# NazirNayal8/RbA

Hardware: AMD Instinct MI355X
Metric: images/sec @1024x2048 Swin-B-1dl (RbA inference hot path) (higher is better)
Workload: dtype f32 (f16x3 split-MFMA GEMMs, fp32 accumulate)

## Files before the change

include/rba_hip.h:

```cpp
#ifndef RBA_HIP_H
#define RBA_HIP_H

#include <stdint.h>

#ifdef __cplusplus
extern "C" {
#endif

int rba_hip_version(void);

int rba_set_concurrent_streams(int n);

int rba_reduce_f32(const float* mask, const float* cls_prob, float* rba, float* sem_seg, int32_t* argmax,
                   int Q, int K, int64_t HW, int score_mode, void* stream);

int rba_reduce_ws_f32(const float* mask, const float* cls_prob, float* rba, float* sem_seg, int32_t* argmax, int Q, int K,
                      int64_t HW, int score_mode, void* workspace, void* stream);

int rba_reduce_up4_f32(const float* mask_lowres, const float* cls_prob, float* rba, float* sem_seg,
                       int32_t* argmax, int Q, int K, int h, int w, int crop_h, int crop_w, int score_mode, void* stream);

int rba_reduce_bwd_workspace_f32(int Q, int K, int64_t HW, int64_t* bytes);
int rba_reduce_bwd_f32(const float* mask, const float* cls_prob, const float* grad_score,
                       float* grad_mask , float* grad_prob ,
// ... 183 lines not shown

int rba_split_linear_f16x3_gn_moments_f32(const float* x, const void* weight_packed, const float* bias, float* out, int64_t M, int N, int K,
                                          int rows_per_image, int G, float* moments, void* stream);
int rba_conv3x3_nhwc_f16x3_split_in_gn_moments_f32(const void* x_frag, const void* weight_packed, const float* bias, float* out, int B, int H,
                                                   int W, int C, int N, int G, float* moments, void* stream);
int rba_group_norm_nhwc_merge_f32(const float* moments, float* mr, int B, int G, int splits, float eps, void* stream);

int rba_patch_im2col_u8(const uint8_t* image, float* out, int h, int w, int Hp, int Wp, const float* mean, const float* std, void* stream);
int rba_patch_im2col_f32(const float* image, float* out, int h, int w, int Hp, int Wp, const float* mean, const float* std, void* stream);

int rba_gaussian_blur_f32(const float* in, float* out, int H, int W, int kernel_size, float sigma, void* stream);

int rba_quad_mean_f32(const float* v, float* out, int64_t rows, int S, void* stream);
int rba_softmax_drop_last_f32(const float* logits, float* prob, int64_t rows, int K1, void* stream);

int rba_threshold_u8(const float* score, uint8_t* out, int64_t n, float threshold, void* stream);
int rba_morph3x3_u8(const uint8_t* in, uint8_t* out, int H, int W, int dilate, void* stream);
int rba_ccl4_roots_i32(const uint8_t* mask, int32_t* roots, int H, int W, void* stream);

int rba_bn_relu_conv1x1_f32(const float* x, const float* scale, const float* shift, const float* weight, const float* bias, float* out,
                            int B, int C, int O, int64_t P, void* stream);
int rba_resample_bilinear_ac_f32(const float* x, float* out, int C, int h, int w, int H, int W, void* stream);

typedef struct {
  const float* x_add;
  const void* packed;
  const float* bias;
  float* out;
  int N;
  int ld_out;
  int act;
} rba_token_linear_problem;
int rba_token_linear_pack_f16x2(const float* weight, void* packed, int N, int K, void* stream);
int rba_token_linear_f32(const float* x, const float* x_add, const void* packed, const float* bias, const float* residual,
                         const float* ln_weight, const float* ln_bias, float ln_eps, float* out, int64_t M, int N, int K, int act,
                         void* stream);
int rba_token_linear_multi_f32(const float* x, const rba_token_linear_problem* problems, int n_problems, int64_t M, int K, void* stream);

#define RBA_TTA_MAX_VIEWS 16
typedef struct {
  const float* sem[RBA_TTA_MAX_VIEWS];
  int h[RBA_TTA_MAX_VIEWS];
  int w[RBA_TTA_MAX_VIEWS];
  int flip[RBA_TTA_MAX_VIEWS];
} rba_tta_views;
int rba_tta_merge_f32(const rba_tta_views* views , int A, int K, int H, int W, int score_mode, float* score, float* sem_seg ,
                      int32_t* argmax , void* stream);

int rba_resize_u8_pil_bilinear(const uint8_t* in , uint8_t* out , uint8_t* tmp , int C, int h, int w,
                               int H, int W, const int32_t* kx, const int32_t* bx, int ksize_x, const int32_t* ky, const int32_t* by, int ksize_y,
                               int flip, void* stream);

int rba_confusion_accum(const int32_t* pred, const void* gt, int gt_bytes , int64_t n_pixels, int K,
                        int ignore_label , const uint8_t* lut , int64_t* conf ,
                        int64_t* bad , void* stream);

typedef struct {
  int enabled;
  int brightness;
  float beta;
  int order;
  int contrast;
  float contrast_alpha;
  int saturation;
  float saturation_alpha;
  int hue;
  int hue_delta;
} rba_train_view_color;
typedef struct {
// ... 25 lines not shown
```

rba_amd/_lib.py:

```python
import ctypes
import os

_HERE = os.path.dirname(os.path.abspath(__file__))
LIB_PATH = os.environ.get("RBA_HIP_LIB") or os.path.join(_HERE, "csrc", "librba_hip.so")
KNOBS_LIB_PATH = os.path.join(_HERE, "csrc", "librba_hip_knobs.so")

_i = ctypes.c_int
_i64 = ctypes.c_int64
_vp = ctypes.c_void_p

SIGNATURES = {
    "rba_hip_version": [],
    "rba_set_concurrent_streams": [_i],
    "rba_reduce_f32": [_vp, _vp, _vp, _vp, _vp, _i, _i, _i64, _i, _vp],
    "rba_reduce_ws_f32": [_vp, _vp, _vp, _vp, _vp, _i, _i, _i64, _i, _vp, _vp],
    "rba_reduce_up4_f32": [_vp, _vp, _vp, _vp, _vp, _i, _i, _i, _i, _i, _i, _i, _vp],
    "rba_reduce_bwd_workspace_f32": [_i, _i, _i64, _vp],
    "rba_reduce_bwd_f32": [_vp, _vp, _vp, _vp, _vp, _i, _i, _i64, _i, _vp, _i64, _vp],
    "rba_sem_seg_bwd_f32": [_vp, _vp, _vp, _vp, _vp, _i, _i, _i64, _vp, _i64, _vp],
    "rba_resample_bilinear_f32": [_vp, _vp, _vp, _i, _i, _i, _i, _i, _vp],
    "rba_ms_deform_attn_fwd_f32": [_vp, _vp, _vp, _vp, _vp, _vp, _i, _i, _i, _i, _i, _i, _i, _vp],
    "rba_ms_deform_attn_fwd_f64": [_vp, _vp, _vp, _vp, _vp, _vp, _i, _i, _i, _i, _i, _i, _i, _vp],
    "rba_ms_deform_attn_bwd_f32": [_vp, _vp, _vp, _vp, _vp, _vp, _vp, _vp, _vp, _i, _i, _i, _i, _i, _i, _i, _vp],
    "rba_ms_deform_attn_bwd_f64": [_vp, _vp, _vp, _vp, _vp, _vp, _vp, _vp, _vp, _i, _i, _i, _i, _i, _i, _i, _vp],
# ... 52 lines not shown
    "rba_swin_mlp_fused_ln_f16x3_f32": [_vp, _vp, _vp, ctypes.c_float, _vp, _vp, _vp, _vp, _i64, _i, _i, _vp],
    "rba_split_linear_f16x3_gelu_split_out": [_vp, _i, _vp, _vp, _vp, _i64, _i, _i, _vp],
    "rba_split_linear_nchw_out_f32": [_vp, _vp, _vp, _vp, _i64, _i, _i, _i, _vp],
    "rba_split_linear_nchw_out_f16x3_f32": [_vp, _vp, _vp, _vp, _i64, _i, _i, _i, _vp],
    "rba_split_linear_f16x3_gn_moments_f32": [_vp, _vp, _vp, _vp, _i64, _i, _i, _i, _i, _vp, _vp],
    "rba_conv3x3_nhwc_f16x3_split_in_gn_moments_f32": [_vp, _vp, _vp, _vp, _i, _i, _i, _i, _i, _i, _vp, _vp],
    "rba_group_norm_nhwc_merge_f32": [_vp, _vp, _i, _i, _i, ctypes.c_float, _vp],
    "rba_split_linear_nchw_out_gn_f16x3_f32": [_vp, _vp, _vp, _vp, _i, _i, _vp, _vp, _vp, _i64, _i, _i, _i, _vp],
    "rba_split_linear_nchw_out_gn_rows_f16x3_f32": [_vp, _vp, _vp, _vp, _i, _i, _vp, _i64, _vp, _i, _vp, _vp, _i, _i, _i, _i, _i, _vp],
    "rba_compose_query_operand_f16x2": [_vp, _vp, _vp, _vp, _vp, _i, _i, _i, _i, _vp],
    "rba_conv3x3_nhwc_f32": [_vp, _vp, _vp, _vp, _i, _i, _i, _i, _i, _vp],
    "rba_conv3x3_nhwc_f16x3_f32": [_vp, _vp, _vp, _vp, _i, _i, _i, _i, _i, _vp],
    "rba_conv3x3_nhwc_f16x3_split_in_f32": [_vp, _vp, _vp, _vp, _i, _i, _i, _i, _i, _vp],
    "rba_resample_bilinear_nhwc_split_out_f32": [_vp, _vp, _vp, _i, _i, _i, _i, _i, _i64, _vp],
    "rba_patch_im2col_u8": [_vp, _vp, _i, _i, _i, _i, _vp, _vp, _vp],
    "rba_patch_im2col_f32": [_vp, _vp, _i, _i, _i, _i, _vp, _vp, _vp],
    "rba_group_norm_nhwc_workspace_bytes": [_i, _i, _i, _i],
    "rba_group_norm_nhwc_f32": [_vp, _vp, _vp, _vp, _vp, _i, _i, _i, _i, ctypes.c_float, _i, _vp],
    "rba_resample_bilinear_nhwc_f32": [_vp, _vp, _vp, _i, _i, _i, _i, _i, _vp],
    "rba_bn_relu_conv1x1_f32": [_vp, _vp, _vp, _vp, _vp, _vp, _i, _i, _i, _i64, _vp],
    "rba_resample_bilinear_ac_f32": [_vp, _vp, _i, _i, _i, _i, _i, _vp],
    "rba_gaussian_blur_f32": [_vp, _vp, _i, _i, _i, ctypes.c_float, _vp],
    "rba_quad_mean_f32": [_vp, _vp, _i64, _i, _vp],
    "rba_softmax_drop_last_f32": [_vp, _vp, _i64, _i, _vp],
    "rba_threshold_u8": [_vp, _vp, _i64, ctypes.c_float, _vp],
    "rba_morph3x3_u8": [_vp, _vp, _i, _i, _i, _vp],
    "rba_ccl4_roots_i32": [_vp, _vp, _i, _i, _vp],
    "rba_add_layer_norm_f32": [_vp, _vp, _vp, _vp, _vp, _vp, _vp, _i64, _i, ctypes.c_float, _vp],
    "rba_add_layer_norm_frag_f32": [_vp, _vp, _vp, _vp, _vp, _vp, _vp, _i64, _i, ctypes.c_float, _vp],
    "rba_merge_layer_norm_f32": [_vp, _vp, _vp, _vp, _i, _i, _i, _i, ctypes.c_float, _vp],
    "rba_group_norm_workspace_bytes": [_i, _i, _i, _i],
    "rba_group_norm_f32": [_vp, _vp, _vp, _vp, _vp, _i, _i, _i, _i, ctypes.c_float, _i, _vp],
    "rba_token_linear_pack_f16x2": [_vp, _vp, _i, _i, _vp],
    "rba_token_linear_f32": [_vp, _vp, _vp, _vp, _vp, _vp, _vp, ctypes.c_float, _vp, _i64, _i, _i, _i, _vp],
    "rba_token_linear_multi_f32": [_vp, _vp, _i, _i64, _i, _vp],
}

class TokenLinearProblem(ctypes.Structure):
    _fields_ = [("x_add", ctypes.c_void_p), ("packed", ctypes.c_void_p), ("bias", ctypes.c_void_p), ("out", ctypes.c_void_p),
                ("N", ctypes.c_int), ("ld_out", ctypes.c_int), ("act", ctypes.c_int)]


TTA_MAX_VIEWS = 16


class TtaViews(ctypes.Structure):
    _fields_ = [("sem", ctypes.c_void_p * TTA_MAX_VIEWS), ("h", ctypes.c_int * TTA_MAX_VIEWS), ("w", ctypes.c_int * TTA_MAX_VIEWS),
                ("flip", ctypes.c_int * TTA_MAX_VIEWS)]


class TrainViewColor(ctypes.Structure):
    _fields_ = [("enabled", ctypes.c_int), ("brightness", ctypes.c_int), ("beta", ctypes.c_float), ("order", ctypes.c_int),
                ("contrast", ctypes.c_int), ("contrast_alpha", ctypes.c_float), ("saturation", ctypes.c_int), ("saturation_alpha", ctypes.c_float),
                ("hue", ctypes.c_int), ("hue_delta", ctypes.c_int)]


TRAIN_VIEW_POINTERS = ("img", "lab", "lut", "obj", "objmask", "kx", "bx", "ky", "by", "ny", "nx", "image", "sem_seg", "outlier_mask", "hist")
TRAIN_VIEW_INTS = ("h", "w", "bh", "bw", "py", "px", "new_h", "new_w", "ksize_x", "ksize_y", "y0", "x0", "ch", "cw", "flip", "pad_h", "pad_w",
                   "ignore_label", "ood_label")


class TrainView(ctypes.Structure):
    _fields_ = ([(n, ctypes.c_void_p) for n in TRAIN_VIEW_POINTERS] + [(n, ctypes.c_int) for n in TRAIN_VIEW_INTS] + [("color", TrainViewColor)])


EXPECTED_ABI = 191

# ... 81 lines not shown
```

rba_amd/csrc/swin_window_attn.hip:

```cpp
#include <stdlib.h>
#include "common.h"
#include "../../include/rba_hip.h"

namespace {

constexpr int CH = 16;

template <int HD>
__global__ __launch_bounds__(256) void swin_window_attn_kernel(const float* __restrict__ qkv, const float* __restrict__ qkv_bias,
                                                               const float* __restrict__ bias, float* __restrict__ out,
                                                               int H, int W, int Hp, int Wp, int nH, int ws, int shift, float scale) {
  extern __shared__ __attribute__((aligned(16))) float lds[];
  const int N = ws * ws;
  float* Ks = lds;
  float* Vs = lds + N * HD;
  int* rid = reinterpret_cast<int*>(lds + 2 * N * HD);
  const int wx = blockIdx.x, wy = blockIdx.y;
  const int h = blockIdx.z % nH, b = blockIdx.z / nH;
  const int C = nH * HD;
  const int64_t tok_stride = 3 * (int64_t)C;
  const float* qkv_b = qkv + (int64_t)b * H * W * tok_stride;

  for (int i = threadIdx.x; i < N * (HD / 4); i += blockDim.x) {
    const int t = i / (HD / 4), d4 = i % (HD / 4);
// ... 258 lines not shown

template <int NT, int WAVES>
int launch_mfma(const float* qkv, const float* qkv_bias, const float* bias, const float* bias_frag, float* out, int B, int H,
                int W, int Hp, int Wp, int nH, int ws, int shift, float scale, hipStream_t st) {
  const size_t shm = (size_t)(2 * NT * 16 * 36) * sizeof(float) + (size_t)(2 * NT * 16) * sizeof(int);
  const dim3 grid(Wp / ws, Hp / ws, B * nH), block(64 * WAVES);
  if (bias_frag)
    hipLaunchKernelGGL((swin_window_attn_mfma_kernel<NT, WAVES, true>), grid, block, shm, st, qkv, qkv_bias, bias_frag, out,
                       H, W, Hp, Wp, nH, ws, shift, scale);
  else
    hipLaunchKernelGGL((swin_window_attn_mfma_kernel<NT, WAVES, false>), grid, block, shm, st, qkv, qkv_bias, bias, out,
                       H, W, Hp, Wp, nH, ws, shift, scale);
  return rba_launch_status();
}

__global__ void swin_bias_fragments_kernel(const float* __restrict__ bias, float* __restrict__ frag, int nH, int N, int NT) {
  const int64_t total = (int64_t)nH * NT * NT * 256;
  for (int64_t i = (int64_t)blockIdx.x * blockDim.x + threadIdx.x; i < total; i += (int64_t)gridDim.x * blockDim.x) {
    const int r = (int)(i & 3), lane = (int)((i >> 2) & 63);
    int64_t j = i >> 8;
    const int c = (int)(j % NT); j /= NT;
    const int strip = (int)(j % NT);
    const int h = (int)(j / NT);
    const int q = strip * 16 + (lane & 15), k = c * 16 + 4 * (lane >> 4) + r;
    frag[i] = (q < N && k < N) ? bias[((int64_t)h * N + q) * N + k] : 0.f;
  }
}

}

#include "swin_window_attn_h3.h"

RBA_KNOB(rba_k5_wpe, 6);

namespace {
template <int NT, int WAVES>
int launch_h3(const float* qkv, const float* qkv_bias, const float* bias, const float* bias_frag, float* out, int B, int H, int W,
              int Hp, int Wp, int nH, int ws, int shift, float scale, hipStream_t st, bool split_out = false) {
  const size_t shm = (size_t)(4 * NT * 16 * 64) + (size_t)(2 * NT * 16) * sizeof(int);
  const dim3 grid(Wp / ws, Hp / ws, B * nH), block(64 * WAVES);
#define K5H_LAUNCH(FRAG, SOUT, WPE, BIAS) hipLaunchKernelGGL((swin_window_attn_h3_kernel<NT, WAVES, FRAG, SOUT, WPE>), grid, block, shm, st, qkv, qkv_bias, BIAS, out, H, W, Hp, Wp, nH, ws, shift, scale)
  const int w = rba_k5_wpe;
  if (split_out && !bias_frag) return (int)hipErrorInvalidValue;
  if (split_out) {
    if (w == 5) K5H_LAUNCH(true, true, 5, bias_frag); else if (w == 7) K5H_LAUNCH(true, true, 7, bias_frag); else K5H_LAUNCH(true, true, 6, bias_frag);
  } else if (bias_frag) {
    if (w == 5) K5H_LAUNCH(true, false, 5, bias_frag); else if (w == 7) K5H_LAUNCH(true, false, 7, bias_frag); else K5H_LAUNCH(true, false, 6, bias_frag);
  } else {
    if (w == 5) K5H_LAUNCH(false, false, 5, bias); else if (w == 7) K5H_LAUNCH(false, false, 7, bias); else K5H_LAUNCH(false, false, 6, bias);
  }
#undef K5H_LAUNCH
  return rba_launch_status();
}

}

extern "C" int64_t rba_swin_bias_fragments_elems(int nH, int ws) {
  if (nH <= 0 || ws <= 0 || ws * ws > 256) return 0;
  const int64_t NT = (ws * ws + 15) / 16;
  return (int64_t)nH * NT * NT * 256;
}

extern "C" int rba_swin_bias_fragments_f32(const float* bias, float* frag, int nH, int ws, void* stream) {
  RBA_CHECK_ARG(bias && frag && nH >= 1 && ws >= 1 && ws * ws <= 256);
  rba_begin();
  const int N = ws * ws, NT = (N + 15) / 16;
  const int64_t total = (int64_t)nH * NT * NT * 256;
  hipLaunchKernelGGL(swin_bias_fragments_kernel, dim3((unsigned)((total + 255) / 256)), dim3(256), 0, (hipStream_t)stream, bias,
                     frag, nH, N, NT);
  return rba_launch_status();
}

extern "C" int rba_swin_window_attn_f32(const float* qkv, const float* qkv_bias, const float* bias, const float* bias_frag,
                                        float* out, int B, int H, int W, int nH, int hd, int ws, int shift, void* stream) {
// ... 42 lines not shown
```

rba_amd/csrc/swin_window_attn_h3.h:

```cpp
#pragma once

#ifdef K5H_TIMING
#define K5H_DBG_PARAM , unsigned long long* __restrict__ dbg
#define K5H_STAMP(i)                                                                                                              \
  do {                                                                                                                            \
    __builtin_amdgcn_sched_barrier(0);                                                                                            \
    if ((threadIdx.x & 63) == 0)                                                                                                  \
      dbg[((((int64_t)blockIdx.z * gridDim.y + blockIdx.y) * gridDim.x + blockIdx.x) * WAVES + (threadIdx.x >> 6)) * 12 + (i)] = wall_clock64(); \
    __builtin_amdgcn_sched_barrier(0);                                                                                            \
  } while (0)
#define K5H_WAIT_VM() __builtin_amdgcn_s_waitcnt(0x0070 | 0x0F00 | 0xC000 * 0)
#define K5H_SINK(x) asm volatile("" ::"s"(__builtin_amdgcn_readfirstlane(__builtin_bit_cast(int, (x)))))
#elif defined(K5H_ABLATE)
#define K5H_DBG_PARAM , int ablate
#define K5H_STAMP(i)
#define K5H_WAIT_VM()
#define K5H_SINK(x)
#else
#define K5H_DBG_PARAM
#define K5H_STAMP(i)
#define K5H_WAIT_VM()
#define K5H_SINK(x)
#endif

namespace {

typedef _Float16 k5h_f16x8 __attribute__((ext_vector_type(8)));
typedef _Float16 k5h_f16x2 __attribute__((ext_vector_type(2)));
typedef __fp16 k5h_h4 __attribute__((__vector_size__(4 * sizeof(__fp16))));
typedef uint32_t k5h_u32x4 __attribute__((ext_vector_type(4)));

template <bool SCALED>
__device__ __forceinline__ void k5h_split2(float a, float b, uint32_t& h, uint32_t& l) {
  const k5h_f16x2 hv = {(_Float16)a, (_Float16)b};
  h = __builtin_bit_cast(uint32_t, hv);
  const float m = SCALED ? -2048.0f : -1.0f;
  const float a2 = SCALED ? a * 2048.0f : a, b2 = SCALED ? b * 2048.0f : b;
  uint32_t r;
  asm("v_fma_mixlo_f16 %0, %1, %2, %3 op_sel_hi:[1,0,0]" : "=v"(r) : "v"(h), "v"(m), "v"(a2));
  asm("v_fma_mixhi_f16 %0, %1, %2, %3 op_sel:[1,0,0] op_sel_hi:[1,0,0]" : "+v"(r) : "v"(h), "v"(m), "v"(b2));
  l = r;
}

template <int NT, int WAVES, bool FRAG, bool SOUT = false, int WPE = 5>
__global__ __launch_bounds__(64 * WAVES) __attribute__((amdgpu_waves_per_eu(WPE, 8))) void swin_window_attn_h3_kernel(
    const float* __restrict__ qkv, const float* __restrict__ qkv_bias, const float* __restrict__ bias, float* __restrict__ out,
    int H, int W, int Hp, int Wp, int nH, int ws, int shift, float scale K5H_DBG_PARAM) {
  K5H_STAMP(0);
#ifdef K5H_ABLATE
  if (((ablate >> 3) & 0xff) && ((((blockIdx.z * gridDim.y + blockIdx.y) * gridDim.x + blockIdx.x) >> 8) & 1)) {
    const unsigned long long t0 = wall_clock64();
    while (wall_clock64() - t0 < (unsigned long long)(((ablate >> 3) & 0xff) * 50)) __builtin_amdgcn_s_sleep(4);
  }
#endif
  constexpr int HD = 32, NP = NT * 16, PL = NP * 64;
  if (NT == 9) ws = 12;
  extern __shared__ __attribute__((aligned(16))) unsigned char k5h_lds[];
  unsigned char* Kh = k5h_lds;
  int* tok = reinterpret_cast<int*>(k5h_lds + 4 * PL);
  int* rid = tok + NP;
  const int N = NT == 9 ? 144 : ws * ws;
  int wx = blockIdx.x, wy = blockIdx.y, hz = blockIdx.z;
#ifdef K5H_ABLATE
  if (ablate & 0x4000) {
    const int L = (blockIdx.z * gridDim.y + blockIdx.y) * gridDim.x + blockIdx.x;
    const int hh = L % nH, wl = L / nH;
    wx = wl % (int)gridDim.x;
    wy = (wl / (int)gridDim.x) % (int)gridDim.y;
    hz = (wl / (int)(gridDim.x * gridDim.y)) * nH + hh;
  }
#endif
  const bool need_mask = shift > 0 && (wy == (int)gridDim.y - 1 || wx == (int)gridDim.x - 1);
  const int h = hz % nH, b = hz / nH;
  const int C = nH * HD;
  const int64_t tok_stride = 3 * (int64_t)C;
  const float* qkv_b = qkv + (int64_t)b * H * W * tok_stride;
  const float* qb = qkv_bias + h * HD;

  constexpr int NIT = (NP * (HD / 4) + 64 * WAVES - 1) / (64 * WAVES);
  float4 kk4[NIT], vv4[NIT];
  int tkv[NIT], rgv[NIT];
#pragma unroll
  for (int it = 0; it < NIT; ++it) {
    const int i = threadIdx.x + it * 64 * WAVES;
    const int t = i >> 3, d4 = i & 7;
    kk4[it] = vv4[it] = make_float4(0.f, 0.f, 0.f, 0.f);
    tkv[it] = -2;
    rgv[it] = -1;
    if (i < NP * (HD / 4) && t < N) {
      const int r = wy * ws + t / ws, c = wx * ws + t % ws;
      int rr = r + shift, cc = c + shift;
      rr = rr >= Hp ? rr - Hp : rr;
      cc = cc >= Wp ? cc - Wp : cc;
#ifdef K5H_ABLATE
      if (ablate & 2) rr = H;
#endif
      if (rr < H && cc < W) {
        tkv[it] = rr * W + cc;
        const float* p = qkv_b + (int64_t)tkv[it] * tok_stride + h * HD + d4 * 4;
        kk4[it] = *reinterpret_cast<const float4*>(p + C);
        vv4[it] = *reinterpret_cast<const float4*>(p + 2 * C);
      } else {
        tkv[it] = -1;
        kk4[it] = *reinterpret_cast<const float4*>(qb + C + d4 * 4);
        vv4[it] = *reinterpret_cast<const float4*>(qb + 2 * C + d4 * 4);
      }
      const int hid = r < Hp - ws ? 0 : (r < Hp - shift ? 1 : 2);
      const int wid = c < Wp - ws ? 0 : (c < Wp - shift ? 1 : 2);
      rgv[it] = hid * 3 + wid;
    }
  }
  float4 q_a = make_float4(0.f, 0.f, 0.f, 0.f), q_b = q_a;
  {
    const int qt0 = (threadIdx.x >> 6) * 16 + (threadIdx.x & 15), kq = (threadIdx.x & 63) >> 4;
    if ((threadIdx.x >> 6) < NT && qt0 < N) {
      const int r = wy * ws + qt0 / ws, c = wx * ws + qt0 % ws;
      int rr = r + shift, cc = c + shift;
      rr = rr >= Hp ? rr - Hp : rr;
      cc = cc >= Wp ? cc - Wp : cc;
#ifdef K5H_ABLATE
      if (ablate & 2) rr = H;
#endif
      const float4* p = (rr < H && cc < W) ? reinterpret_cast<const float4*>(qkv_b + (int64_t)(rr * W + cc) * tok_stride + h * HD + kq * 8)
                                           : reinterpret_cast<const float4*>(qb + kq * 8);
      q_a = p[0];
      q_b = p[1];
    }
  }
  K5H_STAMP(1);
  K5H_WAIT_VM();
  K5H_STAMP(2);
#pragma unroll
  for (int it = 0; it < NIT; ++it) {
    const int i = threadIdx.x + it * 64 * WAVES;
    if (i >= NP * (HD / 4)) break;
    const int t = i >> 3, d4 = i & 7;
    uint32_t h0, l0, h1, l1;
    const int tq = (t >> 2) & 3;
    const int perm = (0x1320 >> (4 * tq)) & 3;
    k5h_split2<false>(kk4[it].x, kk4[it].y, h0, l0);
    k5h_split2<false>(kk4[it].z, kk4[it].w, h1, l1);
    const int ko = t * 64 + (((d4 >> 1) ^ perm) * 16) + (d4 & 1) * 8;
    *reinterpret_cast<uint2*>(Kh + ko) = make_uint2(h0, h1);
    *reinterpret_cast<uint2*>(Kh + PL + ko) = make_uint2(l0, l1);
    k5h_split2<true>(vv4[it].x, vv4[it].y, h0, l0);
    k5h_split2<true>(vv4[it].z, vv4[it].w, h1, l1);
    const int vo = t * 64 + (((d4 >> 2) ^ (tq & 1)) * 32) + (d4 & 3) * 8;
    *reinterpret_cast<uint2*>(Kh + 2 * PL + vo) = make_uint2(h0, h1);
    *reinterpret_cast<uint2*>(Kh + 3 * PL + vo) = make_uint2(l0, l1);
    if (d4 == 0) { tok[t] = tkv[it]; rid[t] = rgv[it]; }
  }
  K5H_STAMP(3);
  __syncthreads();
  K5H_STAMP(4);

  const int lane = threadIdx.x & 63, wave = threadIdx.x >> 6;
  const int l15 = lane & 15, kk = lane >> 4;
  const bool vec_bias = (N & 3) == 0;
  const int kfrag = l15 * 64 + ((kk ^ ((0x1320 >> (4 * ((l15 >> 2) & 3))) & 3)) * 16);
  const int vfrag = (4 * kk + (l15 >> 2)) * 64 + (l15 & 3) * 8;
// ... 196 lines not shown
```

rba_amd/csrc/token_linear.hip:

```cpp
#include "common.h"
#include "../../include/rba_hip.h"

namespace {

typedef _Float16 tl_f16x8 __attribute__((ext_vector_type(8)));
typedef float tl_f32x4 __attribute__((ext_vector_type(4)));

struct TlProblem {
  const float* x_add;
  const rba_u32x4* wp;
  const float* bias;
  float* out;
  int N;
  int ld;
  int act;
};
struct TlProblems {
  TlProblem p[3];
};

__global__ void token_linear_pack_kernel(const float* __restrict__ w, rba_u32x4* __restrict__ packed, int N, int K) {
  const int KB = K >> 5;
  const int64_t total = (int64_t)((N + 15) >> 4) * KB * 128;
  for (int64_t i = (int64_t)blockIdx.x * blockDim.x + threadIdx.x; i < total; i += (int64_t)gridDim.x * blockDim.x) {
// ... 205 lines not shown
        for (int r = 0; r < 4; ++r) y[r] = (val[rt][i][r] - mean[rt]) * rstd * g[r] + be[r];
        *reinterpret_cast<f32x4*>(p.out + (int64_t)row[rt] * p.N + n) = y;
      }
    }
  }
}

RBA_KNOB(rba_token_rt, 0);

template <bool LN>
int launch_token_linear(const float* x, const TlProblems& ps, int nprob, const float* residual, const float* ln_w, const float* ln_b, float eps,
                        int M, int K, hipStream_t st) {
  int nmax = 0;
  for (int i = 0; i < nprob; ++i) nmax = ps.p[i].N > nmax ? ps.p[i].N : nmax;
  const int ctw = (((nmax + 15) >> 4) + TLW - 1) / TLW;
  const bool two = rba_token_rt == 2 || (rba_token_rt == 0 && K >= 512 && M >= 4096);
  const dim3 grid((unsigned)((M + (two ? 31 : 15)) / (two ? 32 : 16)), (unsigned)nprob);
#define RBA_TL(C)                                                                                                                     \
  if (two) hipLaunchKernelGGL((token_linear_kernel<C, LN, 2>), grid, dim3(64 * TLW), 0, st, x, ps, residual, ln_w, ln_b, eps, M, K);   \
  else hipLaunchKernelGGL((token_linear_kernel<C, LN, 1>), grid, dim3(64 * TLW), 0, st, x, ps, residual, ln_w, ln_b, eps, M, K)
  switch (ctw) {
    case 1: RBA_TL(1); break;
    case 2: RBA_TL(2); break;
    case 3: RBA_TL(3); break;
    case 4: RBA_TL(4); break;
    default: return (int)hipErrorInvalidValue;
  }
#undef RBA_TL
  return rba_launch_status();
}

inline bool tl_aligned(const void* p) { return (reinterpret_cast<uintptr_t>(p) & 15) == 0; }

}

extern "C" {

int rba_token_linear_pack_f16x2(const float* weight, void* packed, int N, int K, void* stream) {
  RBA_CHECK_ARG(weight && packed && N >= 1 && K >= 32 && K % 32 == 0 && tl_aligned(packed));
  rba_begin();
  const int64_t total = (int64_t)((N + 15) >> 4) * (K >> 5) * 128;
  const int blocks = (int)((total + 255) / 256 < 4096 ? (total + 255) / 256 : 4096);
  hipLaunchKernelGGL(token_linear_pack_kernel, dim3(blocks), dim3(256), 0, (hipStream_t)stream, weight, reinterpret_cast<rba_u32x4*>(packed), N, K);
  return rba_launch_status();
}

int rba_token_linear_f32(const float* x, const float* x_add, const void* packed, const float* bias, const float* residual,
                         const float* ln_weight, const float* ln_bias, float ln_eps, float* out, int64_t M, int N, int K, int act,
                         void* stream) {
  RBA_CHECK_ARG(x && packed && out && M >= 0 && M < ((int64_t)1 << 31) - 16 && N >= 1 && N <= 256 && K >= 32 && K % 32 == 0);
  RBA_CHECK_ARG(act == 0 || act == 2);
  RBA_CHECK_ARG(tl_aligned(x) && tl_aligned(x_add) && tl_aligned(packed) && tl_aligned(out) && tl_aligned(bias) && N % 4 == 0);
  const bool ln = ln_weight != nullptr;
  RBA_CHECK_ARG(!ln || (residual && ln_bias && N % 16 == 0 && act == 0 && tl_aligned(residual) && tl_aligned(ln_weight) && tl_aligned(ln_bias)));
  RBA_CHECK_ARG(ln || !residual);
  if (M == 0) return 0;
  rba_begin();
  TlProblems ps{};
  ps.p[0] = TlProblem{x_add, reinterpret_cast<const rba_u32x4*>(packed), bias, out, N, N, act};
  if (ln) return launch_token_linear<true>(x, ps, 1, residual, ln_weight, ln_bias, ln_eps, (int)M, K, (hipStream_t)stream);
  return launch_token_linear<false>(x, ps, 1, nullptr, nullptr, nullptr, 0.f, (int)M, K, (hipStream_t)stream);
}

int rba_token_linear_multi_f32(const float* x, const rba_token_linear_problem* problems, int n_problems, int64_t M, int K, void* stream) {
  RBA_CHECK_ARG(x && problems && n_problems >= 1 && n_problems <= 3 && M >= 0 && M < ((int64_t)1 << 31) - 16 && K >= 32 && K % 32 == 0 && tl_aligned(x));
  TlProblems ps{};
  for (int i = 0; i < n_problems; ++i) {
    const rba_token_linear_problem& q = problems[i];
    RBA_CHECK_ARG(q.packed && q.out && q.N >= 1 && q.N <= 256 && q.N % 4 == 0 && q.ld_out >= q.N && q.ld_out % 4 == 0 && (q.act == 0 || q.act == 2));
    RBA_CHECK_ARG(tl_aligned(q.x_add) && tl_aligned(q.packed) && tl_aligned(q.bias) && tl_aligned(q.out));
    ps.p[i] = TlProblem{q.x_add, reinterpret_cast<const rba_u32x4*>(q.packed), q.bias, q.out, q.N, q.ld_out, q.act};
  }
  if (M == 0) return 0;
  rba_begin();
  return launch_token_linear<false>(x, ps, n_problems, nullptr, nullptr, nullptr, 0.f, (int)M, K, (hipStream_t)stream);
}

}
```

rba_amd/ops.py:

```python
import contextlib
import ctypes
import threading
import functools
import math
import os

import torch

from . import _lib
from ._lib import RbaHipError
from .lru import derived


def _stream():
    return torch.cuda.current_stream().cuda_stream


def _launch(name, *args, stream=None):
    code = getattr(_lib.load(), name)(*args, torch.cuda.current_stream().cuda_stream if stream is None else stream)
    if code:
        _lib.check(code, name)


def _query(name, *args):
# ... 1389 lines not shown
    _vec(bias, "bias", N, optional=True)
    splits = H * W // 128
    out = torch.empty((B, H, W, N), dtype=torch.float32, device=x.device)
    mom = torch.empty((B, num_groups, splits, 3), dtype=torch.float32, device=x.device)
    _launch("rba_conv3x3_nhwc_f16x3_split_in_gn_moments_f32", xp, _p(planes), _p(bias), _p(out), B, H, W, C, N, int(num_groups), _p(mom))
    return out, _merge_gn_moments(mom, B, int(num_groups), splits, eps)


def split_linear_nchw_out_takes_gn(planes, rows_per_image, K, num_groups):
    return planes.dtype == torch.float16 and rows_per_image % 128 == 0 and K % num_groups == 0 and (K // num_groups) % 4 == 0 and K % 32 == 0


@_hip_op
def split_linear_nchw_out_gn(x, mr, weight, bias_gn, num_groups, relu, planes, bias, rows_per_image, out_features=None):
    _chk(x, "x", dim=2)
    _chk(mr, "mr", dim=3)
    M, K = x.shape
    N, _ = _packed(planes, K, out_features, bf16x6=False)
    if rows_per_image < 1 or M % rows_per_image or not split_linear_nchw_out_takes_gn(planes, rows_per_image, K, num_groups):
        raise RbaHipError("split_linear_nchw_out_gn needs x [B*P, K], P % 128 == 0 and (K / G) % 4 == 0")
    B = M // rows_per_image
    if tuple(mr.shape) != (B, num_groups, 2):
        raise RbaHipError("mr must be [B, G, 2]")
    _vec(weight, "weight", K)
    _vec(bias_gn, "bias_gn", K)
    _vec(bias, "bias", N, optional=True)
    out = torch.empty((B, N, rows_per_image), dtype=torch.float32, device=x.device)
    _launch("rba_split_linear_nchw_out_gn_f16x3_f32", _p(x), _p(mr), _p(weight), _p(bias_gn), int(num_groups), int(bool(relu)), _p(planes), _p(bias), _p(out),
            M, N, K, rows_per_image)
    return out


COMPOSED_MASK_HEAD = os.environ.get("RBA_COMPOSED_MASK_HEAD", "1") != "0"


class RowIndex:
    __slots__ = ("data", "rows_per_image")

    def __init__(self, data, rows_per_image):
        self.data, self.rows_per_image = data, rows_per_image


def row_index(idx, rows_per_image):
    if not isinstance(idx, torch.Tensor) or not idx.is_cuda or idx.dtype not in (torch.int32, torch.int64) or idx.dim() != 2 or idx.numel() == 0:
        raise RbaHipError("row_index needs a HIP int32 / int64 tensor [B, R]")
    lo, hi = int(idx.min()), int(idx.max())
    if lo < 0 or hi >= rows_per_image:
        raise RbaHipError(f"row_index: values must lie in [0, {rows_per_image}), got [{lo}, {hi}]")
    return RowIndex(idx.to(torch.int32).contiguous(), int(rows_per_image))


def _image_planes(planes, K, out_features, B):
    if planes.dim() != 7:
        return _packed(planes, K, out_features, bf16x6=False)[0], 0
    _chk(planes, "planes", dtype=torch.float16, dim=7)
    if planes.shape[0] != B:
        raise RbaHipError(f"per-image planes must be [B = {B}, ...], got {tuple(planes.shape)}")
    return _packed(planes[0], K, out_features, bf16x6=False)[0], planes.stride(0) * 2


@_hip_op
def split_linear_nchw_out_gn_rows(x, mr, weight, bias_gn, num_groups, relu, planes, bias, rows_per_image, out_features=None, rows=None):
    _chk(x, "x", dim=2)
    _chk(mr, "mr", dim=3)
    M, K = x.shape
    P = int(rows_per_image)
# ... 100 lines not shown

def _token_planes(lin):
    w = lin.weight

    def build():
        w2 = w.detach().contiguous()
        _chk(w2, "weight", dim=2)
        N, K = w2.shape
        packed = torch.empty((((N + 15) // 16) * (K // 32) * 128, 4), dtype=torch.int32, device=w.device)
        _launch("rba_token_linear_pack_f16x2", _p(w2), _p(packed), N, K)
        return packed

    return derived(lin, "token_planes", (w,), build)


@_hip_op
def token_linear(x, lin, x_add=None, use_bias=True, relu=False, residual=None, norm=None):
    _chk(x, "x")
    N, K = lin.weight.shape
    if x.shape[-1] != K or not token_linear_ok(N, K):
        raise RbaHipError("token_linear: x [..., K] with K % 32 == 0, N <= 256 and the f16x3 mode (see token_linear_ok)")
    M = x.numel() // K
    _shaped(x_add, "x_add", x.shape, optional=True)
    bias = _vec(lin.bias if use_bias else None, "bias", N, optional=True)
    if (residual is None) != (norm is None):
        raise RbaHipError("token_linear: residual and norm come together")
    ln_w, ln_b, ln_eps, act = 0, 0, 0.0, 2 if relu else 0
    if norm is not None:
        _chk(residual, "residual")
        if tuple(residual.shape) != tuple(x.shape[:-1]) + (N,) or N % 16 or relu or norm.weight.numel() != N:
            raise RbaHipError("token_linear(norm=...): residual [..., N], N % 16 == 0, no activation")
        ln_w, ln_b, ln_eps = _p(norm.weight), _p(norm.bias), float(norm.eps)
    out = torch.empty(tuple(x.shape[:-1]) + (N,), dtype=torch.float32, device=x.device)
    _launch("rba_token_linear_f32", _p(x), _p(x_add), _p(_token_planes(lin)), _p(bias), _p(residual), ln_w, ln_b, ln_eps, _p(out), M, N, K, act)
    return out


@_hip_op
def token_linear_multi(x, specs):
    _chk(x, "x")
    K = x.shape[-1]
    M = x.numel() // K if K else 0
    lead = tuple(x.shape[:-1])
    if not 1 <= len(specs) <= 3:
        raise RbaHipError("token_linear_multi: one to three problems")
    arr = (_lib.TokenLinearProblem * len(specs))()
    outs, keep = [], []
    for i, (lin, x_add, out, col0, relu) in enumerate(specs):
        N, K_ = lin.weight.shape
        if K_ != K or not token_linear_ok(N, K) or N % 4:
            raise RbaHipError("token_linear_multi: weights [N <= 256, N % 4 == 0, K] with x's K % 32 == 0 (see token_linear_ok)")
        _shaped(x_add, "x_add", x.shape, optional=True)
        _vec(lin.bias, "bias", N, optional=True)
        if out is None:
            out, col0 = torch.empty(lead + (N,), dtype=torch.float32, device=x.device), 0
        else:
            _chk(out, "out")
            if tuple(out.shape[:-1]) != lead or col0 % 4 or col0 + N > out.shape[-1] or out.shape[-1] % 4:
                raise RbaHipError("token_linear_multi: out [..., ld] with ld % 4 == 0 and a column slice col0 % 4 == 0 inside it")
        planes = _token_planes(lin)
        keep.append(planes)
        arr[i] = _lib.TokenLinearProblem(_p(x_add) or None, _p(planes), _p(lin.bias) or None, out.data_ptr() + 4 * col0, N, out.shape[-1], 2 if relu else 0)
        outs.append(out)
    _launch("rba_token_linear_multi_f32", _p(x), ctypes.byref(arr), len(specs), M, K)
    return outs


# ... 177 lines not shown
```

Measured before the change: 151.6.

## Add split-K token linear path and 32-bit-offset gather in Swin window attention

Adds a split-K MFMA kernel plus a separate reduce+bias+residual+LayerNorm finish kernel for token_linear when M is small, N=256 and K>=1024, so the GEMM fills more of the GPU. Partial sums go to a workspace that the host sizes through a new query function. It also adds a GATHER32 variant of the Swin window-attention load that uses 32-bit byte offsets and a row-strided thread mapping for full 12x12 windows, and uses inline -1.0 constants in the unscaled fma_mix path. The costs are extra workspace traffic, one more launch, and a gather path that only covers specific shapes.

After: 152.2, median of 6. Within noise of the previous version (+0.4%).

```diff
diff --git a/include/rba_hip.h b/include/rba_hip.h
--- a/include/rba_hip.h
+++ b/include/rba_hip.h
@@ -239,9 +239,10 @@
   int act;
 } rba_token_linear_problem;
 int rba_token_linear_pack_f16x2(const float* weight, void* packed, int N, int K, void* stream);
+int64_t rba_token_linear_workspace_bytes(int64_t M, int N, int K, int has_ln, int has_x_add);
 int rba_token_linear_f32(const float* x, const float* x_add, const void* packed, const float* bias, const float* residual,
                          const float* ln_weight, const float* ln_bias, float ln_eps, float* out, int64_t M, int N, int K, int act,
-                         void* stream);
+                         void* workspace, int64_t workspace_bytes, void* stream);
 int rba_token_linear_multi_f32(const float* x, const rba_token_linear_problem* problems, int n_problems, int64_t M, int K, void* stream);
 
 #define RBA_TTA_MAX_VIEWS 16
diff --git a/rba_amd/_lib.py b/rba_amd/_lib.py
--- a/rba_amd/_lib.py
+++ b/rba_amd/_lib.py
@@ -108,7 +108,8 @@
     "rba_group_norm_workspace_bytes": [_i, _i, _i, _i],
     "rba_group_norm_f32": [_vp, _vp, _vp, _vp, _vp, _i, _i, _i, _i, ctypes.c_float, _i, _vp],
     "rba_token_linear_pack_f16x2": [_vp, _vp, _i, _i, _vp],
-    "rba_token_linear_f32": [_vp, _vp, _vp, _vp, _vp, _vp, _vp, ctypes.c_float, _vp, _i64, _i, _i, _i, _vp],
+    "rba_token_linear_workspace_bytes": [_i64, _i, _i, _i, _i],
+    "rba_token_linear_f32": [_vp, _vp, _vp, _vp, _vp, _vp, _vp, ctypes.c_float, _vp, _i64, _i, _i, _i, _vp, _i64, _vp],
     "rba_token_linear_multi_f32": [_vp, _vp, _i, _i64, _i, _vp],
 }
 
diff --git a/rba_amd/csrc/swin_window_attn.hip b/rba_amd/csrc/swin_window_attn.hip
--- a/rba_amd/csrc/swin_window_attn.hip
+++ b/rba_amd/csrc/swin_window_attn.hip
@@ -314,6 +314,7 @@
 #include "swin_window_attn_h3.h"
 
 RBA_KNOB(rba_k5_wpe, 6);
+RBA_KNOB(rba_k5_gather, 0);
 
 namespace {
 template <int NT, int WAVES>
@@ -321,7 +322,12 @@
               int Hp, int Wp, int nH, int ws, int shift, float scale, hipStream_t st, bool split_out = false) {
   const size_t shm = (size_t)(4 * NT * 16 * 64) + (size_t)(2 * NT * 16) * sizeof(int);
   const dim3 grid(Wp / ws, Hp / ws, B * nH), block(64 * WAVES);
-#define K5H_LAUNCH(FRAG, SOUT, WPE, BIAS) hipLaunchKernelGGL((swin_window_attn_h3_kernel<NT, WAVES, FRAG, SOUT, WPE>), grid, block, shm, st, qkv, qkv_bias, BIAS, out, H, W, Hp, Wp, nH, ws, shift, scale)
+  const bool g32 = rba_k5_gather == 0 && (int64_t)H * W * 3 * nH * 32 * (int64_t)sizeof(float) < ((int64_t)1 << 32);
+#define K5H_LAUNCH(FRAG, SOUT, WPE, BIAS)                                                                                                                        \
+  do {                                                                                                                                                           \
+    if (g32) hipLaunchKernelGGL((swin_window_attn_h3_kernel<NT, WAVES, FRAG, SOUT, WPE, true>), grid, block, shm, st, qkv, qkv_bias, BIAS, out, H, W, Hp, Wp, nH, ws, shift, scale); \
+    else hipLaunchKernelGGL((swin_window_attn_h3_kernel<NT, WAVES, FRAG, SOUT, WPE, false>), grid, block, shm, st, qkv, qkv_bias, BIAS, out, H, W, Hp, Wp, nH, ws, shift, scale);   \
+  } while (0)
   const int w = rba_k5_wpe;
   if (split_out && !bias_frag) return (int)hipErrorInvalidValue;
   if (split_out) {
diff --git a/rba_amd/csrc/swin_window_attn_h3.h b/rba_amd/csrc/swin_window_attn_h3.h
--- a/rba_amd/csrc/swin_window_attn_h3.h
+++ b/rba_amd/csrc/swin_window_attn_h3.h
@@ -37,12 +37,17 @@
   const float m = SCALED ? -2048.0f : -1.0f;
   const float a2 = SCALED ? a * 2048.0f : a, b2 = SCALED ? b * 2048.0f : b;
   uint32_t r;
-  asm("v_fma_mixlo_f16 %0, %1, %2, %3 op_sel_hi:[1,0,0]" : "=v"(r) : "v"(h), "v"(m), "v"(a2));
-  asm("v_fma_mixhi_f16 %0, %1, %2, %3 op_sel:[1,0,0] op_sel_hi:[1,0,0]" : "+v"(r) : "v"(h), "v"(m), "v"(b2));
+  if constexpr (SCALED) {
+    asm("v_fma_mixlo_f16 %0, %1, %2, %3 op_sel_hi:[1,0,0]" : "=v"(r) : "v"(h), "v"(m), "v"(a2));
+    asm("v_fma_mixhi_f16 %0, %1, %2, %3 op_sel:[1,0,0] op_sel_hi:[1,0,0]" : "+v"(r) : "v"(h), "v"(m), "v"(b2));
+  } else {
+    asm("v_fma_mixlo_f16 %0, %1, -1.0, %2 op_sel_hi:[1,0,0]" : "=v"(r) : "v"(h), "v"(a2));
+    asm("v_fma_mixhi_f16 %0, %1, -1.0, %2 op_sel:[1,0,0] op_sel_hi:[1,0,0]" : "+v"(r) : "v"(h), "v"(b2));
+  }
   l = r;
 }
 
-template <int NT, int WAVES, bool FRAG, bool SOUT = false, int WPE = 5>
+template <int NT, int WAVES, bool FRAG, bool SOUT = false, int WPE = 5, bool GATHER32 = false>
 __global__ __launch_bounds__(64 * WAVES) __attribute__((amdgpu_waves_per_eu(WPE, 8))) void swin_window_attn_h3_kernel(
     const float* __restrict__ qkv, const float* __restrict__ qkv_bias, const float* __restrict__ bias, float* __restrict__ out,
     int H, int W, int Hp, int Wp, int nH, int ws, int shift, float scale K5H_DBG_PARAM) {
@@ -80,6 +85,56 @@
   constexpr int NIT = (NP * (HD / 4) + 64 * WAVES - 1) / (64 * WAVES);
   float4 kk4[NIT], vv4[NIT];
   int tkv[NIT], rgv[NIT];
+  float4 q_a = make_float4(0.f, 0.f, 0.f, 0.f), q_b = q_a;
+  if constexpr (GATHER32) {
+    static_assert(NT == 9 && WAVES <= NT && (8 * WAVES) % 12 == 0 && (NP * (HD / 4)) % (64 * WAVES) == 0,
+                  "GATHER32: full 12 x 12 windows, a thread's pieces whole window rows apart");
+    constexpr int RSTEP = 8 * WAVES / 12;
+    const uint32_t tokb = 12u * (uint32_t)C;
+    const uint32_t rowb = tokb * (uint32_t)W;
+    const char* kbase = reinterpret_cast<const char*>(qkv_b + h * HD + C);
+    const char* vbase = reinterpret_cast<const char*>(qkv_b + h * HD + 2 * C);
+    const int t0 = threadIdx.x >> 3, d4 = threadIdx.x & 7;
+    const int r0 = wy * 12 + t0 / 12, c = wx * 12 + t0 % 12;
+    int cc = c + shift;
+    cc = cc >= Wp ? cc - Wp : cc;
+    const bool colok = cc < W;
+    const int wid = c < Wp - 12 ? 0 : (c < Wp - shift ? 1 : 2);
+    const uint32_t coff = (uint32_t)cc * tokb + (uint32_t)d4 * 16u;
+#pragma unroll
+    for (int it = 0; it < NIT; ++it) {
+      const int r = r0 + it * RSTEP;
+      int rr = r + shift;
+      rr = rr >= Hp ? rr - Hp : rr;
+#ifdef K5H_ABLATE
+      if (ablate & 2) rr = H;
+#endif
+      if (rr < H && colok) {
+        tkv[it] = rr * W + cc;
+        const uint32_t off = (uint32_t)rr * rowb + coff;
+        kk4[it] = *reinterpret_cast<const float4*>(kbase + off);
+        vv4[it] = *reinterpret_cast<const float4*>(vbase + off);
+      } else {
+        tkv[it] = -1;
+        kk4[it] = *reinterpret_cast<const float4*>(qb + C + d4 * 4);
+        vv4[it] = *reinterpret_cast<const float4*>(qb + 2 * C + d4 * 4);
+      }
+      const int hid = r < Hp - 12 ? 0 : (r < Hp - shift ? 1 : 2);
+      rgv[it] = hid * 3 + wid;
+    }
+    const int qt0 = (threadIdx.x >> 6) * 16 + (threadIdx.x & 15), kq = (threadIdx.x & 63) >> 4;
+    int qr = wy * 12 + qt0 / 12 + shift, qc = wx * 12 + qt0 % 12 + shift;
+    qr = qr >= Hp ? qr - Hp : qr;
+    qc = qc >= Wp ? qc - Wp : qc;
+#ifdef K5H_ABLATE
+    if (ablate & 2) qr = H;
+#endif
+    const float4* p = (qr < H && qc < W) ? reinterpret_cast<const float4*>(reinterpret_cast<const char*>(qkv_b + h * HD) + ((uint32_t)qr * rowb +
+                                                                             (uint32_t)qc * tokb + (uint32_t)kq * 32u))
+                                         : reinterpret_cast<const float4*>(qb + kq * 8);
+    q_a = p[0];
+    q_b = p[1];
+  } else {
 #pragma unroll
   for (int it = 0; it < NIT; ++it) {
     const int i = threadIdx.x + it * 64 * WAVES;
@@ -110,7 +165,6 @@
       rgv[it] = hid * 3 + wid;
     }
   }
-  float4 q_a = make_float4(0.f, 0.f, 0.f, 0.f), q_b = q_a;
   {
     const int qt0 = (threadIdx.x >> 6) * 16 + (threadIdx.x & 15), kq = (threadIdx.x & 63) >> 4;
     if ((threadIdx.x >> 6) < NT && qt0 < N) {
@@ -126,6 +180,7 @@
       q_a = p[0];
       q_b = p[1];
     }
+  }
   }
   K5H_STAMP(1);
   K5H_WAIT_VM();
diff --git a/rba_amd/csrc/token_linear.hip b/rba_amd/csrc/token_linear.hip
--- a/rba_amd/csrc/token_linear.hip
+++ b/rba_amd/csrc/token_linear.hip
@@ -261,6 +261,134 @@
 
 inline bool tl_aligned(const void* p) { return (reinterpret_cast<uintptr_t>(p) & 15) == 0; }
 
+constexpr int TLS_N = 256, TLS_CTW = TLS_N / (16 * TLW), TLS_RT = 2, TLS_MAX_SPLITS = 8;
+
+__global__ __launch_bounds__(64 * TLW) void token_linear_splitk_kernel(const float* __restrict__ x, const rba_u32x4* __restrict__ wp,
+                                                                   float* __restrict__ part, int M, int K, int KBS) {
+  constexpr int CTW = TLS_CTW, RT = TLS_RT, N = TLS_N;
+  const int lane = threadIdx.x & 63, wave = __builtin_amdgcn_readfirstlane(threadIdx.x >> 6);
+  const int t = lane & 15, kb = lane >> 4;
+  const int row0 = blockIdx.x * (16 * RT);
+  int row[RT];
+#pragma unroll
+  for (int rt = 0; rt < RT; ++rt) row[rt] = min(row0 + 16 * rt + t, M - 1);
+  const int KB = K >> 5;
+  const int b0 = blockIdx.y * KBS, b1 = min(b0 + KBS, KB);
+  const int nt0 = wave * CTW;
+  const rba_u32x4* wl = wp + lane;
+
+  tl_f32x4 accm[RT][CTW], accl[RT][CTW];
+#pragma unroll
+  for (int rt = 0; rt < RT; ++rt)
+#pragma unroll
+    for (int i = 0; i < CTW; ++i) accm[rt][i] = accl[rt][i] = (tl_f32x4){0.f, 0.f, 0.f, 0.f};
+
+  constexpr int NS = 3;
+  f32x4 a[NS][RT][2];
+  rba_u32x4 wf[NS][CTW][2];
+  auto loads = [&](int b, int s) {
+    if (b >= b1) return;
+#pragma unroll
+    for (int rt = 0; rt < RT; ++rt) {
+      const float* xa = x + (int64_t)row[rt] * K + 8 * kb + 32 * b;
+      a[s][rt][0] = *reinterpret_cast<const f32x4*>(xa);
+      a[s][rt][1] = *reinterpret_cast<const f32x4*>(xa + 4);
+    }
+#pragma unroll
+    for (int i = 0; i < CTW; ++i) {
+      const rba_u32x4* src = wl + ((int64_t)(nt0 + i) * KB + b) * 128;
+      wf[s][i][0] = src[0];
+      wf[s][i][1] = src[64];
+    }
+  };
+  auto compute = [&](int s) {
+#pragma unroll
+    for (int rt = 0; rt < RT; ++rt) {
+      const f32x4 u = a[s][rt][0], v = a[s][rt][1];
+      rba_u32x4 hp, lp;
+      uint32_t h_, l_;
+      rba_split_f16x2(u.x, u.y, h_, l_); hp.x = h_; lp.x = l_;
+      rba_split_f16x2(u.z, u.w, h_, l_); hp.y = h_; lp.y = l_;
+      rba_split_f16x2(v.x, v.y, h_, l_); hp.z = h_; lp.z = l_;
+      rba_split_f16x2(v.z, v.w, h_, l_); hp.w = h_; lp.w = l_;
+      const tl_f16x8 xh = __builtin_bit_cast(tl_f16x8, hp), xl = __builtin_bit_cast(tl_f16x8, lp);
+#pragma unroll
+      for (int i = 0; i < CTW; ++i) {
+        const tl_f16x8 wh = __builtin_bit_cast(tl_f16x8, wf[s][i][0]);
+        accm[rt][i] = __builtin_amdgcn_mfma_f32_16x16x32_f16(wh, xh, accm[rt][i], 0, 0, 0);
+      }
+#pragma unroll
+      for (int i = 0; i < CTW; ++i) {
+        const tl_f16x8 wh = __builtin_bit_cast(tl_f16x8, wf[s][i][0]), wlo = __builtin_bit_cast(tl_f16x8, wf[s][i][1]);
+        accl[rt][i] = __builtin_amdgcn_mfma_f32_16x16x32_f16(wlo, xh, accl[rt][i], 0, 0, 0);
+        accl[rt][i] = __builtin_amdgcn_mfma_f32_16x16x32_f16(wh, xl, accl[rt][i], 0, 0, 0);
+      }
+    }
+  };
+#pragma unroll
+  for (int s = 0; s < NS - 1; ++s) loads(b0 + s, s);
+  for (int b = b0; b < b1; b += NS) {
+#pragma unroll
+    for (int s = 0; s < NS; ++s) {
+      loads(b + s + NS - 1, (s + NS - 1) % NS);
+      if (b + s < b1) compute(s);
+    }
+  }
+  float* dst = part + (int64_t)blockIdx.y * M * N;
+#pragma unroll
+  for (int rt = 0; rt < RT; ++rt) {
+    if (row0 + 16 * rt + t < M) {
+#pragma unroll
+      for (int i = 0; i < CTW; ++i) {
+        f32x4 v;
+#pragma unroll
+        for (int r = 0; r < 4; ++r) v[r] = fmaf(accl[rt][i][r], 0.00048828125f, accm[rt][i][r]);
+        *reinterpret_cast<f32x4*>(dst + (int64_t)row[rt] * N + 16 * (nt0 + i) + 4 * kb) = v;
+      }
+    }
+  }
+}
+
+__global__ __launch_bounds__(64 * TLW) void token_linear_finish_kernel(const float* __restrict__ part, const float* __restrict__ bias,
+                                                                   const float* __restrict__ residual, const float* __restrict__ ln_w,
+                                                                   const float* __restrict__ ln_b, float eps, float* __restrict__ out, int M, int S) {
+  constexpr int N = TLS_N;
+  const int lane = threadIdx.x & 63;
+  const int m = blockIdx.x * TLW + (threadIdx.x >> 6);
+  if (m >= M) return;
+  const int64_t o = (int64_t)m * N + 4 * lane;
+  f32x4 v = *reinterpret_cast<const f32x4*>(part + o);
+#pragma unroll 4
+  for (int s = 1; s < S; ++s) v = v + *reinterpret_cast<const f32x4*>(part + (int64_t)s * M * N + o);
+  if (bias) v = v + *reinterpret_cast<const f32x4*>(bias + 4 * lane);
+  v = *reinterpret_cast<const f32x4*>(residual + o) + v;
+  float s1 = (v.x + v.y) + (v.z + v.w);
+#pragma unroll
+  for (int d = 1; d < 64; d <<= 1) s1 += __shfl_xor(s1, d, RBA_WAVE);
+  const float mean = s1 / (float)N;
+  float s2 = 0.f;
+#pragma unroll
+  for (int r = 0; r < 4; ++r) {
+    const float d = v[r] - mean;
+    s2 = fmaf(d, d, s2);
+  }
+#pragma unroll
+  for (int d = 1; d < 64; d <<= 1) s2 += __shfl_xor(s2, d, RBA_WAVE);
+  const float rstd = rsqrtf(s2 / (float)N + eps);
+  const f32x4 g = *reinterpret_cast<const f32x4*>(ln_w + 4 * lane), be = *reinterpret_cast<const f32x4*>(ln_b + 4 * lane);
+  f32x4 y;
+#pragma unroll
+  for (int r = 0; r < 4; ++r) y[r] = (v[r] - mean) * rstd * g[r] + be[r];
+  *reinterpret_cast<f32x4*>(out + o) = y;
+}
+
+inline int tl_splitk_slices(int64_t M, int N, int K, bool ln, bool has_add) {
+  if (!ln || has_add || N != TLS_N || K < 1024 || M < 1) return 0;
+  const int64_t rb = (M + 16 * TLS_RT - 1) / (16 * TLS_RT);
+  const int64_t S = 256 / rb < TLS_MAX_SPLITS ? 256 / rb : TLS_MAX_SPLITS;
+  return S >= 3 ? (int)S : 0;
+}
+
 }
 
 extern "C" {
@@ -276,7 +404,7 @@
 
 int rba_token_linear_f32(const float* x, const float* x_add, const void* packed, const float* bias, const float* residual,
                          const float* ln_weight, const float* ln_bias, float ln_eps, float* out, int64_t M, int N, int K, int act,
-                         void* stream) {
+                         void* workspace, int64_t workspace_bytes, void* stream) {
   RBA_CHECK_ARG(x && packed && out && M >= 0 && M < ((int64_t)1 << 31) - 16 && N >= 1 && N <= 256 && K >= 32 && K % 32 == 0);
   RBA_CHECK_ARG(act == 0 || act == 2);
   RBA_CHECK_ARG(tl_aligned(x) && tl_aligned(x_add) && tl_aligned(packed) && tl_aligned(out) && tl_aligned(bias) && N % 4 == 0);
@@ -287,8 +415,24 @@
   rba_begin();
   TlProblems ps{};
   ps.p[0] = TlProblem{x_add, reinterpret_cast<const rba_u32x4*>(packed), bias, out, N, N, act};
+  const int S = workspace ? tl_splitk_slices(M, N, K, ln, x_add != nullptr) : 0;
+  if (S) {
+    RBA_CHECK_ARG(tl_aligned(workspace) && workspace_bytes >= (int64_t)S * M * N * (int64_t)sizeof(float));
+    hipStream_t st = (hipStream_t)stream;
+    float* part = reinterpret_cast<float*>(workspace);
+    const int KB = K >> 5, KBS = (KB + S - 1) / S;
+    hipLaunchKernelGGL(token_linear_splitk_kernel, dim3((unsigned)((M + 16 * TLS_RT - 1) / (16 * TLS_RT)), (unsigned)S), dim3(64 * TLW), 0, st, x,
+                       reinterpret_cast<const rba_u32x4*>(packed), part, (int)M, K, KBS);
+    hipLaunchKernelGGL(token_linear_finish_kernel, dim3((unsigned)((M + TLW - 1) / TLW)), dim3(64 * TLW), 0, st, part, bias, residual, ln_weight,
+                       ln_bias, ln_eps, out, (int)M, S);
+    return rba_launch_status();
+  }
   if (ln) return launch_token_linear<true>(x, ps, 1, residual, ln_weight, ln_bias, ln_eps, (int)M, K, (hipStream_t)stream);
   return launch_token_linear<false>(x, ps, 1, nullptr, nullptr, nullptr, 0.f, (int)M, K, (hipStream_t)stream);
+}
+
+int64_t rba_token_linear_workspace_bytes(int64_t M, int N, int K, int has_ln, int has_x_add) {
+  return (int64_t)tl_splitk_slices(M, N, K, has_ln != 0, has_x_add != 0) * M * N * (int64_t)sizeof(float);
 }
 
 int rba_token_linear_multi_f32(const float* x, const rba_token_linear_problem* problems, int n_problems, int64_t M, int K, void* stream) {
diff --git a/rba_amd/ops.py b/rba_amd/ops.py
--- a/rba_amd/ops.py
+++ b/rba_amd/ops.py
@@ -1445,6 +1445,7 @@
 
 
 COMPOSED_MASK_HEAD = os.environ.get("RBA_COMPOSED_MASK_HEAD", "1") != "0"
+SMALL_KERNEL_PATHS = os.environ.get("RBA_SMALL_KERNEL_PATHS", "1") != "0"
 
 
 class RowIndex:
@@ -1611,7 +1612,10 @@
             raise RbaHipError("token_linear(norm=...): residual [..., N], N % 16 == 0, no activation")
         ln_w, ln_b, ln_eps = _p(norm.weight), _p(norm.bias), float(norm.eps)
     out = torch.empty(tuple(x.shape[:-1]) + (N,), dtype=torch.float32, device=x.device)
-    _launch("rba_token_linear_f32", _p(x), _p(x_add), _p(_token_planes(lin)), _p(bias), _p(residual), ln_w, ln_b, ln_eps, _p(out), M, N, K, act)
+    ws_bytes = _query("rba_token_linear_workspace_bytes", M, N, K, int(norm is not None), int(x_add is not None)) if SMALL_KERNEL_PATHS else 0
+    ws = _scratch(ws_bytes, x.device) if ws_bytes else None
+    _launch("rba_token_linear_f32", _p(x), _p(x_add), _p(_token_planes(lin)), _p(bias), _p(residual), ln_w, ln_b, ln_eps, _p(out), M, N, K, act,
+            _p(ws), ws_bytes)
     return out
 
 
```
